# irfanfadhullah/unet_zoo

Measured on AMD Instinct MI355X. Metric: images/sec (fwd+bwd) at B=16 3x256x256, 1/2/4/8 MI355X, higher is better.
Workload: dtype bf16; 1 GPU; unet train step (zero_grad+fwd+BCE+bwd+clip+AdamW), B=16/GPU 3x256x256, random-init weights; global_batch=16, parallelism=dp1

## Files before the change

unet_zoo_amd/csrc/uz_eltwise.hip:

```cpp
#include "uz_common.h"

namespace {

template <typename T> __device__ __forceinline__ void load_f(const T* p, float* f) {
  const Vec16<T> v = ld16(p);
#pragma unroll
  for (int i = 0; i < ElemTraits<T>::VEC; ++i) f[i] = (float)v.v[i];
}
template <typename T> __device__ __forceinline__ void store_f(T* p, const float* f) {
  Vec16<T> v;
#pragma unroll
  for (int i = 0; i < ElemTraits<T>::VEC; ++i) v.v[i] = (T)f[i];
  st16(p, v);
}

template <int EW>
__global__ __launch_bounds__(1024) void bn_finalize_kernel(
    const float* __restrict__ part, int grid_m, int C, double count, const float* __restrict__ gamma,
    const float* __restrict__ beta, float eps, float momentum, float* running_mean,
    float* running_var, float* scale, float* shift, float* mean, float* invstd) {
  constexpr int NG = 1024 / EW;
  __shared__ double sh[2][NG][EW + 1];
  const int cl = threadIdx.x % EW, g = threadIdx.x / EW;
  const int c = blockIdx.x * EW + cl;
// ... 52 lines not shown
constexpr int FIN_SH_DOUBLES = 2 * 128 * 9;

template <int EW>
__device__ __forceinline__ void fin_row_sums(const float* __restrict__ part, int rows, int C, int blk, int tid, double* sh) {
  constexpr int NG = 1024 / EW, LD = EW + 1, GS = 256 / EW;
  const int cl = tid % EW, g0 = tid / EW, c = blk * EW + cl;
  double a1[4] = {0.0, 0.0, 0.0, 0.0}, a2[4] = {0.0, 0.0, 0.0, 0.0};
  if (c < C) {
    for (int r0 = g0; r0 < rows; r0 += NG) {
      float x1[4], x2[4];
#pragma unroll
      for (int k = 0; k < 4; ++k) {
        const int r = r0 + k * GS;
        const int rc = r < rows ? r : 0;
        x1[k] = part[((size_t)rc * 2 + 0) * C + c];
        x2[k] = part[((size_t)rc * 2 + 1) * C + c];
      }
#pragma unroll
      for (int k = 0; k < 4; ++k)
        if (r0 + k * GS < rows) {
          a1[k] += (double)x1[k];
          a2[k] += (double)x2[k];
        }
    }
  }
#pragma unroll
  for (int k = 0; k < 4; ++k) {
    sh[(0 * NG + g0 + k * GS) * LD + cl] = a1[k];
    sh[(1 * NG + g0 + k * GS) * LD + cl] = a2[k];
  }
  __syncthreads();
#pragma unroll
  for (int st = NG / 2; st > 0; st >>= 1) {
    for (int v = tid; v < st * EW; v += 256) {
      const int vl = v % EW, g = v / EW;
      sh[(0 * NG + g) * LD + vl] += sh[(0 * NG + g + st) * LD + vl];
      sh[(1 * NG + g) * LD + vl] += sh[(1 * NG + g + st) * LD + vl];
    }
    __syncthreads();
  }
}

struct BnFin {
  const float* part;
  int rows, ew;
  double count;
  const float *gamma, *beta;
  float eps, momentum;
  float *running_mean, *running_var;
  float* vec;
  double* sums;
  float *dgamma, *dbeta;
  int* flag;
};

#ifndef UZ_FIN_SLEEP
#define UZ_FIN_SLEEP 4
#endif
template <typename V> __device__ __forceinline__ void fin_store(V* p, V v) {
  __hip_atomic_store(p, v, __ATOMIC_RELAXED, __HIP_MEMORY_SCOPE_AGENT);
}
template <typename V> __device__ __forceinline__ V fin_load(const V* p) {
  return __hip_atomic_load(const_cast<V*>(p), __ATOMIC_RELAXED, __HIP_MEMORY_SCOPE_AGENT);
}
__device__ __forceinline__ void fin_publish(int* flag, int tid) {
  asm volatile("s_waitcnt vmcnt(0)" ::: "memory");
  __syncthreads();
  if (tid == 0) __hip_atomic_fetch_add(flag, 1, __ATOMIC_RELAXED, __HIP_MEMORY_SCOPE_AGENT);
}
__device__ __forceinline__ void fin_wait(int* flag, int nfin, int tid) {
  if (tid == 0)
    while (__hip_atomic_load(flag, __ATOMIC_RELAXED, __HIP_MEMORY_SCOPE_AGENT) < nfin) __builtin_amdgcn_s_sleep(UZ_FIN_SLEEP);
  __syncthreads();
}

template <int EW>
__device__ __forceinline__ void fin_forward(const BnFin& f, int C, int blk, int tid, double* sh) {
  constexpr int NG = 1024 / EW, LD = EW + 1;
  fin_row_sums<EW>(f.part, f.rows, C, blk, tid, sh);
  const int c = blk * EW + tid;
  if (tid < EW && c < C) {
    const double t1 = sh[(0 * NG) * LD + tid], t2 = sh[(1 * NG) * LD + tid];
    const double m = t1 / f.count;
    double var = t2 / f.count - m * m;
    if (var < 0.0) var = 0.0;
    const double istd = 1.0 / sqrt(var + (double)f.eps);
    fin_store(f.vec + c, (float)((double)f.gamma[c] * istd));
    fin_store(f.vec + C + c, (float)((double)f.beta[c] - m * (double)f.gamma[c] * istd));
    f.vec[2 * C + c] = (float)m;
    f.vec[3 * C + c] = (float)istd;
    if (f.running_mean != nullptr) {
      const double unbiased = f.count > 1.0 ? var * f.count / (f.count - 1.0) : var;
      f.running_mean[c] = (float)((1.0 - (double)f.momentum) * (double)f.running_mean[c] + (double)f.momentum * m);
      f.running_var[c] = (float)((1.0 - (double)f.momentum) * (double)f.running_var[c] + (double)f.momentum * unbiased);
    }
  }
}

template <int EW>
__device__ __forceinline__ void fin_backward(const BnFin& f, int C, int blk, int tid, double* sh) {
  constexpr int NG = 1024 / EW, LD = EW + 1;
  fin_row_sums<EW>(f.part, f.rows, C, blk, tid, sh);
  const int c = blk * EW + tid;
  if (tid < EW && c < C) {
    const double t1 = sh[(0 * NG) * LD + tid], t2 = sh[(1 * NG) * LD + tid];
    fin_store(f.sums + c, t1);
    fin_store(f.sums + C + c, t2);
    if (f.dgamma != nullptr) {
      f.dbeta[c] = (float)t1;
      f.dgamma[c] = (float)t2;
    }
  }
}

__global__ void bn_eval_scale_kernel(int C, const float* gamma, const float* beta, const float* rm,
                                     const float* rv, float eps, float* scale, float* shift) {
  const int c = blockIdx.x * blockDim.x + threadIdx.x;
  if (c < C) {
    const float istd = 1.0f / sqrtf(rv[c] + eps);
    const float sc = gamma[c] * istd;
    scale[c] = sc;
    shift[c] = beta[c] - rm[c] * sc;
  }
}

template <typename T, bool POOL, bool FIN = false>
__global__ __launch_bounds__(256) void bn_relu_apply_kernel(
    const T* __restrict__ y, int ldy, const float* scale, const float* shift,
    int N, int H, int W, int C, T* __restrict__ act, int lda, T* __restrict__ pooled, int ldp,
    const T* __restrict__ res, int ldr, int pool_ceil, const BnFin fin) {
  const float* fin_tab = nullptr;
  if constexpr (FIN) {
    __shared__ double fin_sh[FIN_SH_DOUBLES];
    const int nfin = (C + fin.ew - 1) / fin.ew;
    if ((int)blockIdx.x < nfin) {
      if (fin.ew == 8) fin_forward<8>(fin, C, blockIdx.x, threadIdx.x, fin_sh);
      else fin_forward<32>(fin, C, blockIdx.x, threadIdx.x, fin_sh);
      fin_publish(fin.flag, threadIdx.x);
    }
    fin_wait(fin.flag, nfin, threadIdx.x);
    float* tab = reinterpret_cast<float*>(fin_sh);
    for (int i = threadIdx.x; i < 2 * C; i += 256) tab[i] = fin_load(fin.vec + i);
    __syncthreads();
    fin_tab = tab;
  }
  constexpr int VEC = ElemTraits<T>::VEC;
  const int CC = C / VEC;
  const bool relu = !(pool_ceil & 2);
  const bool rev = (pool_ceil & 4) != 0;
  pool_ceil &= 1;
  const int Ho = (H + 1) >> 1, Wo = (W + 1) >> 1;
  const int Hp = pool_ceil ? Ho : H >> 1, Wp = pool_ceil ? Wo : W >> 1;
  const long long total = POOL ? (long long)N * Ho * Wo * CC : (long long)N * H * W * CC;
  for (long long idx0 = (long long)blockIdx.x * blockDim.x + threadIdx.x; idx0 < total;
       idx0 += (long long)gridDim.x * blockDim.x) {
    const long long idx = rev ? total - 1 - idx0 : idx0;
    const int cc = (int)(idx % CC);
    const long long u = idx / CC;
    const int c0 = cc * VEC;
    float sc[VEC], sh[VEC];
    if constexpr (FIN) {
#pragma unroll
      for (int i = 0; i < VEC; i += 4) {
        *reinterpret_cast<float4*>(sc + i) = *reinterpret_cast<const float4*>(fin_tab + c0 + i);
        *reinterpret_cast<float4*>(sh + i) = *reinterpret_cast<const float4*>(fin_tab + C + c0 + i);
      }
    } else {
#pragma unroll
      for (int i = 0; i < VEC; i += 4) {
        *reinterpret_cast<float4*>(sc + i) = *reinterpret_cast<const float4*>(scale + c0 + i);
        *reinterpret_cast<float4*>(sh + i) = *reinterpret_cast<const float4*>(shift + c0 + i);
      }
    }
    if constexpr (!POOL) {
      float v[VEC];
      load_f(y + (size_t)u * ldy + c0, v);
#pragma unroll
      for (int i = 0; i < VEC; ++i) {
        v[i] = fmaf(v[i], sc[i], sh[i]);
        if (relu) v[i] = fmaxf(v[i], 0.f);
      }
      if (res != nullptr) {
        float r[VEC];
        load_f(res + (size_t)u * ldr + c0, r);
#pragma unroll
        for (int i = 0; i < VEC; ++i) v[i] += r[i];
      }
      store_f(act + (size_t)u * lda + c0, v);
    } else {
      const int wo = (int)(u % Wo);
      const long long t = u / Wo;
      const int ho = (int)(t % Ho);
      const int img = (int)(t / Ho);
      const size_t p00 = ((size_t)img * H + 2 * ho) * W + 2 * wo;
      float m[VEC];
      bool ok[4];
      size_t pp[4];
      Vec16<T> vr[4], rr[4];
#pragma unroll
      for (int k = 0; k < 4; ++k) {
        ok[k] = 2 * ho + (k >> 1) < H && 2 * wo + (k & 1) < W;
        pp[k] = p00 + (k >> 1) * W + (k & 1);
        vr[k] = ld16(ok[k] ? y + pp[k] * ldy + c0 : y + c0);
        rr[k] = ld16(res != nullptr && ok[k] ? res + pp[k] * ldr + c0 : y + c0);
      }
#pragma unroll
      for (int k = 0; k < 4; ++k) {
        float v[VEC];
#pragma unroll
        for (int i = 0; i < VEC; ++i) {
          v[i] = fmaf((float)vr[k].v[i], sc[i], sh[i]);
          if (relu) v[i] = fmaxf(v[i], 0.f);
          if (res != nullptr) v[i] = (float)(T)(v[i] + (float)rr[k].v[i]);
          m[i] = (k == 0) ? v[i] : (ok[k] ? fmaxf(m[i], v[i]) : m[i]);
        }
        if (ok[k]) store_f(act + pp[k] * lda + c0, v);
      }
      if (ho < Hp && wo < Wp) store_f(pooled + (((size_t)img * Hp + ho) * Wp + wo) * ldp + c0, m);
    }
  }
}

struct BnBwdArgs {
  const void* y;
  const void* g0;
  const void* g1;
  const void* gp;
  void* dy;
  const float* scale;
  const float* shift;
  const float* mean;
  const float* invstd;
  double* sums;
  float* partials;
  float* dgamma;
  float* dbeta;
  double inv_count;
  int N, H, W, C, ldy, ldg0, ldg1, ldgp, lddy, pool_ceil;
  BnFin fin;
};

template <typename T, bool POOL, int PASS, bool FIN = false>
__global__ __launch_bounds__(256) void bn_relu_bwd_kernel(const BnBwdArgs a) {
  constexpr int VEC = ElemTraits<T>::VEC;
  const double* fin_tab = nullptr;
  if constexpr (FIN) {
    static_assert(PASS == 2, "the fused finalize belongs to the apply pass");
    __shared__ double fin_sh[FIN_SH_DOUBLES];
    const int nfin = (a.C + a.fin.ew - 1) / a.fin.ew;
    const int wg = blockIdx.y * gridDim.x + blockIdx.x, tid = threadIdx.y * blockDim.x + threadIdx.x;
    if (wg < nfin) {
      if (a.fin.ew == 8) fin_backward<8>(a.fin, a.C, wg, tid, fin_sh);
      else fin_backward<32>(a.fin, a.C, wg, tid, fin_sh);
      fin_publish(a.fin.flag, tid);
    }
    fin_wait(a.fin.flag, nfin, tid);
    const int cw = blockDim.x * VEC, cb = blockIdx.y * cw;
    for (int i = tid; i < 2 * cw; i += 256) {
      const int which = i / cw, j = i - which * cw;
      fin_sh[i] = cb + j < a.C ? fin_load(a.sums + (size_t)which * a.C + cb + j) : 0.0;
    }
    __syncthreads();
    fin_tab = fin_sh;
  }
  constexpr int NPIX = 4;
  extern __shared__ __attribute__((aligned(16))) float red[];
  const T* __restrict__ y = static_cast<const T*>(a.y);
  const T* __restrict__ g0 = static_cast<const T*>(a.g0);
  const T* __restrict__ g1 = static_cast<const T*>(a.g1);
  const T* __restrict__ gp = static_cast<const T*>(a.gp);
  T* __restrict__ dy = static_cast<T*>(a.dy);
  const int CC = a.C / VEC;
  const int cc = blockIdx.y * blockDim.x + threadIdx.x;
  const bool cok = cc < CC;
  const int c0 = (cok ? cc : 0) * VEC;
  const int Ho = (a.H + 1) >> 1, Wo = (a.W + 1) >> 1;
  const bool norelu = (a.pool_ceil & 2) != 0;
  const int Hp = (a.pool_ceil & 1) ? Ho : a.H >> 1, Wp = (a.pool_ceil & 1) ? Wo : a.W >> 1;
  const long long units = POOL ? (long long)a.N * Ho * Wo : (long long)a.N * a.H * a.W;

  float sc[VEC], sh[VEC], mu[VEC], is[VEC], k0[VEC], k1[VEC];
#pragma unroll
  for (int i = 0; i < VEC; ++i) {
    sc[i] = a.scale[c0 + i];
    sh[i] = a.shift[c0 + i];
    mu[i] = a.mean[c0 + i];
    is[i] = a.invstd[c0 + i];
    if (PASS == 2) {
      if constexpr (FIN) {
        k0[i] = (float)(fin_tab[threadIdx.x * VEC + i] * a.inv_count);
        k1[i] = (float)(fin_tab[blockDim.x * VEC + threadIdx.x * VEC + i] * a.inv_count);
      } else {
        k0[i] = (float)(a.sums[c0 + i] * a.inv_count);
        k1[i] = (float)(a.sums[a.C + c0 + i] * a.inv_count);
      }
    }
  }
  float S0[VEC], S1[VEC];
#pragma unroll
  for (int i = 0; i < VEC; ++i) S0[i] = S1[i] = 0.f;

  const long long ustride = (long long)gridDim.x * blockDim.y;
  const bool rev = (a.pool_ceil & 4) != 0;
  for (long long u0 = (long long)blockIdx.x * blockDim.y + threadIdx.y; u0 < units && cok;
       u0 += (POOL ? 1 : NPIX) * ustride) {
    size_t pix[NPIX];
    bool in[NPIX];
    size_t gpoff = 0;
    bool has_pool = false;
    if constexpr (POOL) {
      const long long u = rev ? units - 1 - u0 : u0;
      const int wo = (int)(u % Wo);
      const long long t = u / Wo;
      const int ho = (int)(t % Ho);
      const int img = (int)(t / Ho);
#pragma unroll
      for (int k = 0; k < NPIX; ++k) {
        const int hh = 2 * ho + (k >> 1), ww = 2 * wo + (k & 1);
        in[k] = hh < a.H && ww < a.W;
        pix[k] = ((size_t)img * a.H + min(hh, a.H - 1)) * a.W + min(ww, a.W - 1);
      }
      has_pool = ho < Hp && wo < Wp;
      gpoff = (((size_t)img * Hp + ho) * Wp + wo) * a.ldgp;
    } else {
#pragma unroll
      for (int k = 0; k < NPIX; ++k) {
        const long long q = u0 + k * ustride;
        in[k] = q < units;
        pix[k] = (size_t)(in[k] ? (rev ? units - 1 - q : q) : units - 1);
      }
    }
#ifndef UZ_BN_BRANCHY
    Vec16<T> yr[NPIX], g0r[NPIX], g1r[NPIX], gpr;
#pragma unroll
    for (int k = 0; k < NPIX; ++k) {
      yr[k] = ld16(y + pix[k] * a.ldy + c0);
      if constexpr (POOL) {
        g0r[k] = ld16(g0 != nullptr ? g0 + pix[k] * a.ldg0 + c0 : y + c0);
        g1r[k] = ld16(g1 != nullptr ? g1 + pix[k] * a.ldg1 + c0 : y + c0);
      } else {
        if (g0 != nullptr) g0r[k] = ld16(g0 + pix[k] * a.ldg0 + c0);
        if (g1 != nullptr) g1r[k] = ld16(g1 + pix[k] * a.ldg1 + c0);
      }
    }
    if constexpr (POOL) gpr = ld16(gp != nullptr ? gp + (has_pool ? gpoff : 0) + c0 : y + c0);
    float yv[NPIX][VEC], gv[NPIX][VEC];
#pragma unroll
    for (int k = 0; k < NPIX; ++k)
#pragma unroll
      for (int i = 0; i < VEC; ++i) {
        yv[k][i] = in[k] ? (float)yr[k].v[i] : 0.f;
        float gsum = g0 != nullptr ? (float)g0r[k].v[i] : 0.f;
        if (g1 != nullptr) gsum += (float)g1r[k].v[i];
        gv[k][i] = in[k] ? gsum : 0.f;
      }
#else
    float yv[NPIX][VEC], gv[NPIX][VEC];
#pragma unroll
    for (int k = 0; k < NPIX; ++k) {
      const size_t p = pix[k];
      if (!in[k]) {
#pragma unroll
        for (int i = 0; i < VEC; ++i) yv[k][i] = gv[k][i] = 0.f;
        continue;
      }
      load_f(y + p * a.ldy + c0, yv[k]);
      if (g0 != nullptr) {
        load_f(g0 + p * a.ldg0 + c0, gv[k]);
      } else {
#pragma unroll
        for (int i = 0; i < VEC; ++i) gv[k][i] = 0.f;
      }
      if (g1 != nullptr) {
        float t[VEC];
        load_f(g1 + p * a.ldg1 + c0, t);
#pragma unroll
        for (int i = 0; i < VEC; ++i) gv[k][i] += t[i];
      }
    }
#endif
    if constexpr (POOL) {
      if (gp != nullptr && has_pool) {
        float gpv[VEC];
#ifndef UZ_BN_BRANCHY
#pragma unroll
        for (int i = 0; i < VEC; ++i) gpv[i] = (float)gpr.v[i];
#else
        load_f(gp + gpoff + c0, gpv);
#endif
#pragma unroll
        for (int i = 0; i < VEC; ++i) {
          float best = fmaf(yv[0][i], sc[i], sh[i]);
          if (!norelu) best = fmaxf(best, 0.f);
          int bk = 0;
#pragma unroll
          for (int k = 1; k < 4; ++k) {
            float v = fmaf(yv[k][i], sc[i], sh[i]);
            if (!norelu) v = fmaxf(v, 0.f);
            if (in[k] && v > best) {
              best = v;
              bk = k;
            }
          }
#pragma unroll
          for (int k = 0; k < 4; ++k) gv[k][i] += (k == bk) ? gpv[i] : 0.f;
        }
      }
    }
#pragma unroll
    for (int k = 0; k < NPIX; ++k) {
      if (!in[k]) continue;
      float out[VEC];
#pragma unroll
      for (int i = 0; i < VEC; ++i) {
        const float pre = fmaf(yv[k][i], sc[i], sh[i]);
        const float dz = (norelu || pre > 0.f) ? gv[k][i] : 0.f;
        const float xh = (yv[k][i] - mu[i]) * is[i];
        if (PASS == 1) {
          S0[i] += dz;
          S1[i] += dz * xh;
        } else {
          out[i] = sc[i] * (dz - k0[i] - xh * k1[i]);
        }
      }
      if (PASS == 2) {
        store_f(dy + pix[k] * a.lddy + c0, out);
      }
    }
  }

  if (PASS == 1) {
    float* mine = red + ((size_t)threadIdx.y * blockDim.x + threadIdx.x) * (2 * VEC);
#pragma unroll
    for (int i = 0; i < VEC; ++i) {
      mine[i] = S0[i];
      mine[VEC + i] = S1[i];
    }
    __syncthreads();
    for (int e = threadIdx.y; e < 2 * VEC; e += blockDim.y) {
      float t = 0.f;
      for (int r = 0; r < (int)blockDim.y; ++r) t += red[((size_t)r * blockDim.x + threadIdx.x) * (2 * VEC) + e];
      if (cok) {
        const int which = e / VEC, ch = c0 + (e % VEC);
        a.partials[((size_t)blockIdx.x * 2 + which) * a.C + ch] = t;
      }
    }
  }
}

struct BnBwdHeadArgs {
  const bf16_t* y;
  bf16_t* dy;
  const float* scale;
  const float* shift;
  const float* mean;
  const float* invstd;
  const double* sums;
  const float* g;
  const float* w;
  double inv_count;
  int P, HW, C, ldy, lddy, rev;
};

template <int KOUT>
__global__ __launch_bounds__(256) void bn_relu_bwd_head_kernel(const BnBwdHeadArgs a) {
  typedef bf16_t T;
  constexpr int VEC = ElemTraits<T>::VEC, NPIX = 4;
  const T* __restrict__ y = a.y;
  const float* __restrict__ g = a.g;
  T* __restrict__ dy = a.dy;
  const int CC = a.C / VEC;
  const int cc = blockIdx.y * blockDim.x + threadIdx.x;
  const bool cok = cc < CC;
  const int c0 = (cok ? cc : 0) * VEC;
  const long long units = a.P;

  float sc[VEC], sh[VEC], mu[VEC], is[VEC], k0[VEC], k1[VEC], wr[KOUT][VEC];
#pragma unroll
  for (int i = 0; i < VEC; ++i) {
    sc[i] = a.scale[c0 + i];
    sh[i] = a.shift[c0 + i];
    mu[i] = a.mean[c0 + i];
    is[i] = a.invstd[c0 + i];
    k0[i] = (float)(a.sums[c0 + i] * a.inv_count);
    k1[i] = (float)(a.sums[a.C + c0 + i] * a.inv_count);
#pragma unroll
    for (int k = 0; k < KOUT; ++k) wr[k][i] = a.w[k * a.C + c0 + i];
  }
  const long long ustride = (long long)gridDim.x * blockDim.y;
  const bool rev = a.rev != 0;
  for (long long u0 = (long long)blockIdx.x * blockDim.y + threadIdx.y; u0 < units && cok; u0 += NPIX * ustride) {
    size_t pix[NPIX];
    bool in[NPIX];
#pragma unroll
    for (int k = 0; k < NPIX; ++k) {
      const long long q = u0 + k * ustride;
      in[k] = q < units;
      pix[k] = (size_t)(in[k] ? (rev ? units - 1 - q : q) : units - 1);
    }
    Vec16<T> yr[NPIX];
    float gq[NPIX][KOUT];
#pragma unroll
    for (int k = 0; k < NPIX; ++k) {
      yr[k] = ld16(y + pix[k] * a.ldy + c0);
      const int p = (int)pix[k];
      const int img = (KOUT == 1) ? 0 : p / a.HW;
      const int hw = p - img * a.HW;
#pragma unroll
      for (int kk = 0; kk < KOUT; ++kk) gq[k][kk] = g[((size_t)img * KOUT + kk) * a.HW + hw];
    }
#pragma unroll
    for (int k = 0; k < NPIX; ++k) {
      if (!in[k]) continue;
      float out[VEC];
#pragma unroll
      for (int i = 0; i < VEC; ++i) {
        float d = 0.f;
#pragma unroll
        for (int kk = 0; kk < KOUT; ++kk) d = fmaf(gq[k][kk], wr[kk][i], d);
        const float gv = (float)(T)d;
        const float yv = (float)yr[k].v[i];
        const float pre = fmaf(yv, sc[i], sh[i]);
        const float dz = pre > 0.f ? gv : 0.f;
        const float xh = (yv - mu[i]) * is[i];
        out[i] = sc[i] * (dz - k0[i] - xh * k1[i]);
      }
      store_f(dy + pix[k] * a.lddy + c0, out);
    }
  }
}

template <int EW>
__global__ __launch_bounds__(1024) void bn_bwd_finalize_kernel(const float* __restrict__ part, int rows,
                                                               int C, double* __restrict__ sums,
                                                               float* dgamma, float* dbeta) {
  constexpr int NG = 1024 / EW;
  __shared__ double sh[2][NG][EW + 1];
  const int cl = threadIdx.x % EW, g = threadIdx.x / EW;
  const int c = blockIdx.x * EW + cl;
  double a1 = 0.0, a2 = 0.0;
  const int cq = c < C ? c : 0;
  for (int r = g; r < rows; r += 4 * NG) {
    float p1[4], p2[4];
#pragma unroll
    for (int k = 0; k < 4; ++k) {
      const int rr = r + k * NG < rows ? r + k * NG : 0;
      p1[k] = part[((size_t)rr * 2 + 0) * C + cq];
      p2[k] = part[((size_t)rr * 2 + 1) * C + cq];
    }
#pragma unroll
    for (int k = 0; k < 4; ++k) asm volatile("" : "+v"(p1[k]), "+v"(p2[k]));
#pragma unroll
    for (int k = 0; k < 4; ++k)
      if (r + k * NG < rows && c < C) {
        a1 += (double)p1[k];
        a2 += (double)p2[k];
      }
  }
  sh[0][g][cl] = a1;
  sh[1][g][cl] = a2;
  __syncthreads();
#pragma unroll
  for (int st = NG / 2; st > 0; st >>= 1) {
    if (g < st) {
      sh[0][g][cl] += sh[0][g + st][cl];
      sh[1][g][cl] += sh[1][g + st][cl];
    }
    __syncthreads();
  }
  if (g == 0 && c < C) {
    const double t1 = sh[0][0][cl], t2 = sh[1][0][cl];
    sums[c] = t1;
    sums[C + c] = t2;
    if (dgamma != nullptr) {
      dbeta[c] = (float)t1;
      dgamma[c] = (float)t2;
    }
  }
}

constexpr int OUTCONV_MAXK = 8;
__host__ __device__ inline int lanes_per_pixel(int chunks) {
  int l = 1;
  while (l < chunks) l <<= 1;
  return l;
}

template <typename T, int KOUT, bool XF = false>
__global__ __launch_bounds__(256) void outconv_fwd_kernel(const T* __restrict__ x, int ldx, int N,
                                                          int HW, int C, const float* __restrict__ w,
                                                          const float* __restrict__ b,
                                                          float* __restrict__ out,
                                                          const float* __restrict__ xf_scale = nullptr,
                                                          const float* __restrict__ xf_shift = nullptr) {
  constexpr int VEC = ElemTraits<T>::VEC;
  const int LPP = lanes_per_pixel(C / VEC);
  const int ppb = blockDim.x / LPP;
  const int sub = threadIdx.x % LPP, pl = threadIdx.x / LPP;
  const bool live = sub < C / VEC;
  const int P = N * HW;
  float wr[KOUT][VEC];
#pragma unroll
  for (int k = 0; k < KOUT; ++k)
#pragma unroll
    for (int i = 0; i < VEC; ++i) wr[k][i] = live ? w[k * C + sub * VEC + i] : 0.f;
  float xsc[VEC], xsh[VEC];
  if constexpr (XF) {
#pragma unroll
    for (int i = 0; i < VEC; ++i) {
      xsc[i] = live ? xf_scale[sub * VEC + i] : 0.f;
      xsh[i] = live ? xf_shift[sub * VEC + i] : 0.f;
    }
  }
  for (int p0 = blockIdx.x * ppb; p0 < P; p0 += gridDim.x * ppb) {
    const int p = p0 + pl;
    float v[VEC];
    if (p < P && live) {
      load_f(x + (size_t)p * ldx + sub * VEC, v);
      if constexpr (XF) {
#pragma unroll
        for (int i = 0; i < VEC; ++i) v[i] = (float)(T)fmaxf(fmaf(v[i], xsc[i], xsh[i]), 0.f);
      }
    } else {
#pragma unroll
      for (int i = 0; i < VEC; ++i) v[i] = 0.f;
    }
    const int img = (KOUT == 1) ? 0 : p / HW;
    const int hw = p - img * HW;
#pragma unroll
    for (int k = 0; k < KOUT; ++k) {
      float s = 0.f;
#pragma unroll
      for (int i = 0; i < VEC; ++i) s = fmaf(v[i], wr[k][i], s);
      for (int o = LPP >> 1; o > 0; o >>= 1) s += __shfl_xor(s, o);
      if (sub == 0 && p < P) out[((size_t)img * KOUT + k) * HW + hw] = s + b[k];
    }
  }
}

template <typename T, int KOUT, bool BNRED = false, bool XNULL = false>
__global__ __launch_bounds__(256) void outconv_bwd_kernel(const T* __restrict__ x, int ldx, int N,
                                                          int HW, int C, const float* __restrict__ w,
                                                          const float* __restrict__ g,
                                                          T* __restrict__ dx, int lddx,
                                                          float* __restrict__ partial, const T* __restrict__ bn_y = nullptr, int ld_bny = 0,
                                                          const float* __restrict__ bn_scale = nullptr, const float* __restrict__ bn_shift = nullptr,
                                                          const float* __restrict__ bn_mean = nullptr, const float* __restrict__ bn_invstd = nullptr,
                                                          float* __restrict__ bnpart = nullptr) {
  constexpr int VEC = ElemTraits<T>::VEC;
// ... 373 lines not shown
      {
        float tv[16];
#pragma unroll
        for (int k = 0; k < 16; ++k) {
          const int r = ty + 4 * k;
          tv[k] = src[(r0 + r < R && c0 + tx < Cc) ? (size_t)(r0 + r) * Cc + c0 + tx : 0];
        }
#pragma unroll
        for (int k = 0; k < 16; ++k) asm volatile("" : "+v"(tv[k]));
#pragma unroll
        for (int k = 0; k < 16; ++k) {
          const int r = ty + 4 * k;
          tile[r][tx] = (r0 + r < R && c0 + tx < Cc) ? tv[k] : 0.f;
        }
      }
      __syncthreads();
      for (int c = ty; c < 64; c += 4)
        if (c0 + c < Cc && r0 + tx < R) dst[(size_t)(c0 + c) * R + r0 + tx] = (T)tile[tx][c];
    }
    return;
  }
  if (it.T == 4 && it.mode == UZ_PACK_CONVT_DGRAD && count == 4LL * it.Co * it.Ci) {
    const int rowlen = 4 * it.Co;
    for (int ci = blockIdx.x; ci < it.Ci; ci += gridDim.x) {
      const float* __restrict__ srow = src + (size_t)ci * rowlen;
      T* __restrict__ drow = dst + (size_t)ci * rowlen;
      for (int k = threadIdx.x; k < rowlen; k += 256) {
        const int t = k / it.Co, co = k - t * it.Co;
        drow[k] = (T)srow[4 * co + t];
      }
    }
    return;
  }
  if (it.T == 4 && it.mode == UZ_PACK_CONVT_FWD && count == 4LL * it.Co * it.Ci) {
    const int R = it.Ci, Cc = 4 * it.Co;
    __shared__ float tile4[64][65];
    const int tr = (R + 63) / 64, tc = (Cc + 63) / 64;
    const int tx = threadIdx.x & 63, ty = threadIdx.x >> 6;
    for (int t = blockIdx.x; t < tr * tc; t += gridDim.x) {
      const int r0 = (t / tc) * 64, c0 = (t % tc) * 64;
      __syncthreads();
      {
        float tv[16];
#pragma unroll
        for (int k = 0; k < 16; ++k) {
          const int r = ty + 4 * k;
          tv[k] = src[(r0 + r < R && c0 + tx < Cc) ? (size_t)(r0 + r) * Cc + c0 + tx : 0];
        }
#pragma unroll
        for (int k = 0; k < 16; ++k) asm volatile("" : "+v"(tv[k]));
#pragma unroll
        for (int k = 0; k < 16; ++k) {
          const int r = ty + 4 * k;
          tile4[r][tx] = (r0 + r < R && c0 + tx < Cc) ? tv[k] : 0.f;
        }
      }
      __syncthreads();
      for (int c = ty; c < 64; c += 4) {
        const int j = c0 + c;
        if (j < Cc && r0 + tx < R) dst[(size_t)((j & 3) * it.Co + (j >> 2)) * R + r0 + tx] = (T)tile4[tx][c];
      }
    }
    return;
  }
  for (long long idx = (long long)blockIdx.x * blockDim.x + threadIdx.x; idx < count;
       idx += (long long)gridDim.x * blockDim.x)
    dst[idx] = (T)pack_element(it.mode, it.src, it.Co, it.Ci, it.T, it.Kpad, idx);
}

template <typename T>
__global__ void im2col3x3_kernel(const float* __restrict__ x, int N, int C, int H, int W, int Kpad,
                                 T* __restrict__ dst, long long total) {
  constexpr int VEC = ElemTraits<T>::VEC;
  const int cpr = Kpad / VEC;
  for (long long idx = (long long)blockIdx.x * blockDim.x + threadIdx.x; idx < total;
       idx += (long long)gridDim.x * blockDim.x) {
    const int ch = (int)(idx % cpr);
    const long long p = idx / cpr;
    const int w0 = (int)(p % W);
    const long long q = p / W;
    const int h0 = (int)(q % H);
    const int img = (int)(q / H);
    Vec16<T> v;
#pragma unroll
    for (int e = 0; e < VEC; ++e) {
      const int k = ch * VEC + e;
      float f = 0.f;
      if (k < 9 * C) {
        const int t = k / C, c = k - t * C;
        const int hh = h0 + t / 3 - 1, ww = w0 + t % 3 - 1;
        if ((unsigned)hh < (unsigned)H && (unsigned)ww < (unsigned)W)
          f = x[(((size_t)img * C + c) * H + hh) * W + ww];
      }
      v.v[e] = (T)f;
    }
    st16(dst + (size_t)p * Kpad + ch * VEC, v);
  }
}

template <typename T, int C>
__global__ __launch_bounds__(256) void im2col3x3_smallc_kernel(const float* __restrict__ x, int N, int H,
                                                               int W, int Kpad, T* __restrict__ dst,
                                                               long long npix) {
  constexpr int VEC = ElemTraits<T>::VEC;
  constexpr int K = 9 * C;
  constexpr int MAXCH = 64 / VEC;
  constexpr int ROWB = MAXCH * 16 + 16;
  __shared__ __attribute__((aligned(16))) char strip[4][64 * ROWB];
  const int nch = Kpad / VEC;
  const int lane = threadIdx.x & 63, wv = threadIdx.x >> 6;
  char* mine = strip[wv];
  for (long long p0 = ((long long)blockIdx.x * blockDim.x + (threadIdx.x & ~63)); p0 < npix;
       p0 += (long long)gridDim.x * blockDim.x) {
    const long long p = p0 + lane;
    float row[K];
    if (p < npix) {
      const int w0 = (int)(p % W);
      const long long q = p / W;
      const int h0 = (int)(q % H);
      const int img = (int)(q / H);
#pragma unroll
      for (int t = 0; t < 9; ++t) {
        const int hh = h0 + t / 3 - 1, ww = w0 + t % 3 - 1;
        const bool ok = (unsigned)hh < (unsigned)H && (unsigned)ww < (unsigned)W;
#pragma unroll
        for (int c = 0; c < C; ++c) row[t * C + c] = ok ? x[(((size_t)img * C + c) * H + hh) * W + ww] : 0.f;
      }
    } else {
#pragma unroll
      for (int k = 0; k < K; ++k) row[k] = 0.f;
    }
#pragma unroll
    for (int ch = 0; ch < MAXCH; ++ch) {
      if (ch < nch) {
        Vec16<T> v;
#pragma unroll
        for (int e = 0; e < VEC; ++e) v.v[e] = (ch * VEC + e < K) ? (T)row[(ch * VEC + e < K) ? ch * VEC + e : 0] : (T)0.f;
        *reinterpret_cast<Vec16<T>*>(mine + lane * ROWB + ch * 16) = v;
      }
    }
    asm volatile("s_waitcnt lgkmcnt(0)" ::: "memory");
    const int total = 64 * nch;
    for (int j = lane; j < total; j += 64) {
      const int px = j / nch, ch = j - px * nch;
      if (p0 + px < npix) {
        const Vec16<T> v = *reinterpret_cast<const Vec16<T>*>(mine + px * ROWB + ch * 16);
        st16(dst + (size_t)(p0 + px) * Kpad + ch * VEC, v);
      }
    }
    asm volatile("s_waitcnt lgkmcnt(0)" ::: "memory");
  }
}

int grid_for(long long total, int block) {
  long long g = (total + block - 1) / block;
  const long long cap = (long long)UZ_NUM_CU * 8;
  if (g > cap) g = cap;
  if (g < 1) g = 1;
  return (int)g;
}


void reduce_shape(int CC, long long units, dim3* grid, dim3* block, int wg_per_cu = 2) {
  int bx = 1;
  while (bx < CC && bx < 64) bx <<= 1;
  const int by = 256 / bx;
  const int gy = (CC + bx - 1) / bx;
  long long gx = (units + by - 1) / by;
  long long cap = (long long)UZ_NUM_CU * wg_per_cu / gy;
  if (cap < 1) cap = 1;
  if (gx > cap) gx = cap;
  if (gx < 1) gx = 1;
  *grid = dim3((unsigned)gx, (unsigned)gy);
  *block = dim3(bx, by);
}

}

extern "C" int uz_bn_finalize(const float* stats_partial, int grid_m, int C, double count,
                              const float* gamma, const float* beta, float eps, float momentum,
                              float* running_mean, float* running_var, float* scale, float* shift,
                              float* mean, float* invstd, void* stream) {
  UZ_REQUIRE(stats_partial && gamma && beta && scale && shift && mean && invstd, "uz_bn_finalize: null");
  UZ_REQUIRE(grid_m > 0 && C > 0 && count > 0, "uz_bn_finalize: bad shape");
  UZ_REQUIRE((running_mean == nullptr) == (running_var == nullptr), "uz_bn_finalize: running stats");
  if (grid_m >= 128 && C <= 512)
    hipLaunchKernelGGL(bn_finalize_kernel<8>, dim3(uz_cdiv(C, 8)), dim3(1024), 0, (hipStream_t)stream,
                       stats_partial, grid_m, C, count, gamma, beta, eps, momentum, running_mean,
                       running_var, scale, shift, mean, invstd);
  else
    hipLaunchKernelGGL(bn_finalize_kernel<32>, dim3(uz_cdiv(C, 32)), dim3(1024), 0, (hipStream_t)stream,
                       stats_partial, grid_m, C, count, gamma, beta, eps, momentum, running_mean,
                       running_var, scale, shift, mean, invstd);
  UZ_LAUNCH_CHECK("uz_bn_finalize");
  return UZ_OK;
}

extern "C" int uz_bn_eval_scale(int C, const float* gamma, const float* beta, const float* running_mean,
                                const float* running_var, float eps, float* scale, float* shift,
                                void* stream) {
  UZ_REQUIRE(C > 0 && gamma && beta && running_mean && running_var && scale && shift, "uz_bn_eval_scale: null");
  hipLaunchKernelGGL(bn_eval_scale_kernel, dim3(uz_cdiv(C, 256)), dim3(256), 0, (hipStream_t)stream, C,
                     gamma, beta, running_mean, running_var, eps, scale, shift);
  UZ_LAUNCH_CHECK("uz_bn_eval_scale");
  return UZ_OK;
}

template <typename T>
static int bn_relu_apply_t(const void* y, int ldy, const float* scale, const float* shift, int N, int H,
                           int W, int C, void* act, int lda, void* pooled, int ldp, const void* res, int ldr,
                           int pool_ceil, hipStream_t s) {
  constexpr int VEC = ElemTraits<T>::VEC;
  if (pooled != nullptr) {
    const long long total = (long long)N * ((H + 1) / 2) * ((W + 1) / 2) * (C / VEC);
    hipLaunchKernelGGL((bn_relu_apply_kernel<T, true>), dim3(grid_for(total, 256)), dim3(256), 0, s,
                       (const T*)y, ldy, scale, shift, N, H, W, C, (T*)act, lda, (T*)pooled, ldp, (const T*)res, ldr, pool_ceil, BnFin{});
  } else {
    const long long total = (long long)N * H * W * (C / VEC);
    hipLaunchKernelGGL((bn_relu_apply_kernel<T, false>), dim3(grid_for(total, 256)), dim3(256), 0, s,
                       (const T*)y, ldy, scale, shift, N, H, W, C, (T*)act, lda, (T*)nullptr, 0, (const T*)res, ldr, pool_ceil & 6, BnFin{});
  }
  UZ_LAUNCH_CHECK("uz_bn_relu_apply");
  return UZ_OK;
}

extern "C" int uz_bn_relu_add_apply(int dtype, const void* y, int ldy, const float* scale, const float* shift,
                                    int N, int H, int W, int C, const void* res, int ldr, void* act, int lda,
                                    void* pooled, int ldp, int pool_ceil, void* stream);

extern "C" int uz_bn_relu_apply(int dtype, const void* y, int ldy, const float* scale, const float* shift,
                                int N, int H, int W, int C, void* act, int lda, void* pooled, int ldp,
                                void* stream) {
  return uz_bn_relu_add_apply(dtype, y, ldy, scale, shift, N, H, W, C, nullptr, 0, act, lda, pooled, ldp, 0, stream);
}

extern "C" int uz_bn_relu_add_apply(int dtype, const void* y, int ldy, const float* scale, const float* shift,
                                    int N, int H, int W, int C, const void* res, int ldr, void* act, int lda,
                                    void* pooled, int ldp, int pool_ceil, void* stream) {
  UZ_REQUIRE(dtype == UZ_F32 || dtype == UZ_BF16, "uz_bn_relu_apply: bad dtype");
  const int vec = dtype == UZ_BF16 ? 8 : 4;
  UZ_REQUIRE(y && scale && shift && act, "uz_bn_relu_apply: null pointer");
  UZ_REQUIRE(N > 0 && H > 0 && W > 0 && C > 0 && C % vec == 0, "uz_bn_relu_apply: C=%d must be a multiple of %d", C, vec);
  UZ_REQUIRE(ldy % vec == 0 && lda % vec == 0 && ldy >= C && lda >= C, "uz_bn_relu_apply: bad ld");
  if (res != nullptr) UZ_REQUIRE(ldr % vec == 0 && ldr >= C, "uz_bn_relu_apply: bad ldr");
  if (pooled != nullptr) {
    UZ_REQUIRE((pool_ceil & 1) || (H >= 2 && W >= 2), "uz_bn_relu_apply: floor-mode pool of a %dx%d map is empty", H, W);
    UZ_REQUIRE(ldp % vec == 0 && ldp >= C, "uz_bn_relu_apply: bad ldp");
  }
  hipStream_t s = (hipStream_t)stream;
  return dtype == UZ_BF16 ? bn_relu_apply_t<bf16_t>(y, ldy, scale, shift, N, H, W, C, act, lda, pooled, ldp, res, ldr, pool_ceil, s)
                          : bn_relu_apply_t<float>(y, ldy, scale, shift, N, H, W, C, act, lda, pooled, ldp, res, ldr, pool_ceil, s);
}

static inline int fin_ew(int rows, int C) { return (rows >= 128 && C <= 512) ? 8 : 32; }

template <typename T>
static int bn_relu_apply_fin_t(const void* y, int ldy, const BnFin& fin, int N, int H, int W, int C, void* act, int lda,
                               void* pooled, int ldp, const void* res, int ldr, int pool_ceil, hipStream_t s, bool* done) {
  constexpr int VEC = ElemTraits<T>::VEC;
  const bool pool = pooled != nullptr;
  const long long total = (pool ? (long long)N * ((H + 1) / 2) * ((W + 1) / 2) : (long long)N * H * W) * (C / VEC);
  const int grid = grid_for(total, 256);
  *done = grid >= (C + fin.ew - 1) / fin.ew && 2 * C <= 2 * FIN_SH_DOUBLES;
  if (!*done) return UZ_OK;
  if (pool)
    hipLaunchKernelGGL((bn_relu_apply_kernel<T, true, true>), dim3(grid), dim3(256), 0, s, (const T*)y, ldy, fin.vec, fin.vec + C, N,
                       H, W, C, (T*)act, lda, (T*)pooled, ldp, (const T*)res, ldr, pool_ceil, fin);
  else
    hipLaunchKernelGGL((bn_relu_apply_kernel<T, false, true>), dim3(grid), dim3(256), 0, s, (const T*)y, ldy, fin.vec, fin.vec + C,
                       N, H, W, C, (T*)act, lda, (T*)nullptr, 0, (const T*)res, ldr, pool_ceil & 6, fin);
  UZ_LAUNCH_CHECK("uz_bn_relu_add_apply_fin");
  return UZ_OK;
}

extern "C" int uz_bn_relu_add_apply_fin(int dtype, const void* y, int ldy, const float* stats_partial, int rows, double count,
                                        const float* gamma, const float* beta, float eps, float momentum, float* running_mean,
                                        float* running_var, float* vec, int* flag, int N, int H, int W, int C, const void* res,
                                        int ldr, void* act, int lda, void* pooled, int ldp, int pool_ceil, void* stream) {
  UZ_REQUIRE(dtype == UZ_F32 || dtype == UZ_BF16, "uz_bn_relu_add_apply_fin: bad dtype");
  const int vecw = dtype == UZ_BF16 ? 8 : 4;
  UZ_REQUIRE(y && act && stats_partial && gamma && beta && vec && flag, "uz_bn_relu_add_apply_fin: null pointer");
  UZ_REQUIRE(rows > 0 && count > 0, "uz_bn_relu_add_apply_fin: bad statistics shape");
  UZ_REQUIRE((running_mean == nullptr) == (running_var == nullptr), "uz_bn_relu_add_apply_fin: running stats");
  UZ_REQUIRE(N > 0 && H > 0 && W > 0 && C > 0 && C % vecw == 0, "uz_bn_relu_add_apply_fin: C=%d must be a multiple of %d", C, vecw);
  UZ_REQUIRE(ldy % vecw == 0 && lda % vecw == 0 && ldy >= C && lda >= C, "uz_bn_relu_add_apply_fin: bad ld");
  if (res != nullptr) UZ_REQUIRE(ldr % vecw == 0 && ldr >= C, "uz_bn_relu_add_apply_fin: bad ldr");
  if (pooled != nullptr) {
    UZ_REQUIRE((pool_ceil & 1) || (H >= 2 && W >= 2), "uz_bn_relu_add_apply_fin: floor-mode pool of a %dx%d map is empty", H, W);
    UZ_REQUIRE(ldp % vecw == 0 && ldp >= C, "uz_bn_relu_add_apply_fin: bad ldp");
  }
  BnFin fin{};
  fin.part = stats_partial; fin.rows = rows; fin.ew = fin_ew(rows, C); fin.count = count;
  fin.gamma = gamma; fin.beta = beta; fin.eps = eps; fin.momentum = momentum;
  fin.running_mean = running_mean; fin.running_var = running_var; fin.vec = vec; fin.flag = flag;
  hipStream_t s = (hipStream_t)stream;
  bool done = false;
  const int rc = dtype == UZ_BF16
      ? bn_relu_apply_fin_t<bf16_t>(y, ldy, fin, N, H, W, C, act, lda, pooled, ldp, res, ldr, pool_ceil, s, &done)
      : bn_relu_apply_fin_t<float>(y, ldy, fin, N, H, W, C, act, lda, pooled, ldp, res, ldr, pool_ceil, s, &done);
  if (rc != UZ_OK || done) return rc;
  const int rc2 = uz_bn_finalize(stats_partial, rows, C, count, gamma, beta, eps, momentum, running_mean, running_var, vec,
                                 vec + C, vec + 2 * C, vec + 3 * C, stream);
  if (rc2 != UZ_OK) return rc2;
  return uz_bn_relu_add_apply(dtype, y, ldy, vec, vec + C, N, H, W, C, res, ldr, act, lda, pooled, ldp, pool_ceil, stream);
}

static int bnbwd_check(const uz_bnbwd_desc* d, const void* g0, const void* g1, const void* gp) {
  UZ_REQUIRE(d != nullptr, "uz_bn_relu_bwd: null descriptor");
  UZ_REQUIRE(d->dtype == UZ_F32 || d->dtype == UZ_BF16, "uz_bn_relu_bwd: bad dtype");
  const int vec = d->dtype == UZ_BF16 ? 8 : 4;
  UZ_REQUIRE(d->N > 0 && d->H > 0 && d->W > 0 && d->C > 0 && d->C % vec == 0, "uz_bn_relu_bwd: bad shape");
  UZ_REQUIRE(d->ldy % vec == 0 && d->ldy >= d->C, "uz_bn_relu_bwd: bad ldy");
  if (g0) UZ_REQUIRE(d->ldg0 % vec == 0 && d->ldg0 >= d->C, "uz_bn_relu_bwd: bad ldg0");
  if (g1) UZ_REQUIRE(d->ldg1 % vec == 0 && d->ldg1 >= d->C, "uz_bn_relu_bwd: bad ldg1");
  if (gp) {
    UZ_REQUIRE(d->ldgp % vec == 0 && d->ldgp >= d->C, "uz_bn_relu_bwd: bad ldgp");
  }
  UZ_REQUIRE(g0 || g1 || gp, "uz_bn_relu_bwd: no incoming gradient");
  return UZ_OK;
}

static void bnbwd_shape(const uz_bnbwd_desc* d, bool pool, dim3* grid, dim3* block, int pass = 1) {
  const int vec = d->dtype == UZ_BF16 ? 8 : 4;
  const long long units = pool ? (long long)d->N * ((d->H + 1) / 2) * ((d->W + 1) / 2) : (long long)d->N * d->H * d->W;
  const int f = uz_tune_flags() & 6;
  reduce_shape(d->C / vec, units, grid, block, pass == 2 ? 8 : (f == 2 ? 8 : f == 4 ? 6 : 4));
}

template <typename T, int PASS, bool FIN = false>
static int bnbwd_launch(const uz_bnbwd_desc* d, const BnBwdArgs& a, bool pool, hipStream_t s) {
  constexpr int VEC = ElemTraits<T>::VEC;
  dim3 grid, block;
  bnbwd_shape(d, pool, &grid, &block, PASS);
  const size_t shm = PASS == 1 ? (size_t)256 * 2 * VEC * sizeof(float) : 0;
  if constexpr (FIN) {
    UZ_REQUIRE((long long)grid.x * grid.y >= (a.C + a.fin.ew - 1) / a.fin.ew && block.x * block.y == 256,
               "uz_bn_relu_bwd_apply_fin: the grid is smaller than the finalize (ask uz_bn_relu_bwd_apply_fin_supported)");
  }
  if (pool) {
    hipLaunchKernelGGL((bn_relu_bwd_kernel<T, true, PASS, FIN>), grid, block, shm, s, a);
  } else {
    hipLaunchKernelGGL((bn_relu_bwd_kernel<T, false, PASS, FIN>), grid, block, shm, s, a);
  }
  UZ_LAUNCH_CHECK("uz_bn_relu_bwd");
  return UZ_OK;
}

static BnBwdArgs bnbwd_args(const uz_bnbwd_desc* d, const void* y, const float* scale, const float* shift,
                            const float* mean, const float* invstd, const void* g0, const void* g1,
                            const void* gp) {
  BnBwdArgs a;
  a.y = y;
  a.g0 = g0;
  a.g1 = g1;
  a.gp = gp;
  a.dy = nullptr;
  a.scale = scale;
  a.shift = shift;
  a.mean = mean;
  a.invstd = invstd;
  a.sums = nullptr;
  a.partials = nullptr;
  a.dgamma = nullptr;
  a.dbeta = nullptr;
  a.inv_count = 0.0;
  a.N = d->N;
  a.H = d->H;
  a.W = d->W;
  a.C = d->C;
  a.ldy = d->ldy;
  a.ldg0 = d->ldg0;
  a.ldg1 = d->ldg1;
  a.ldgp = d->ldgp;
  a.pool_ceil = d->pool_ceil;
  a.lddy = d->lddy;
  a.fin = BnFin{};
  return a;
}

static void bnbwd_finalize(const float* partial, int rows, int C, double* sums, float* dgamma, float* dbeta,
                           hipStream_t s) {
  if (rows >= 128 && C <= 512)
    hipLaunchKernelGGL(bn_bwd_finalize_kernel<8>, dim3(uz_cdiv(C, 8)), dim3(1024), 0, s, partial, rows, C, sums, dgamma, dbeta);
  else
    hipLaunchKernelGGL(bn_bwd_finalize_kernel<32>, dim3(uz_cdiv(C, 32)), dim3(1024), 0, s, partial, rows, C, sums, dgamma, dbeta);
}

extern "C" long long uz_bn_relu_bwd_workspace_bytes(const uz_bnbwd_desc* d, int has_pool_grad) {
  UZ_REQUIRE(d != nullptr && d->C > 0 && d->N > 0 && d->H > 0 && d->W > 0, "uz_bn_relu_bwd_workspace_bytes: bad descriptor");
  UZ_REQUIRE(d->dtype == UZ_F32 || d->dtype == UZ_BF16, "uz_bn_relu_bwd_workspace_bytes: bad dtype");
  dim3 grid, block;
  bnbwd_shape(d, has_pool_grad != 0, &grid, &block);
  return (long long)grid.x * 2 * d->C * (long long)sizeof(float);
}

extern "C" int uz_bn_relu_bwd_reduce(const uz_bnbwd_desc* d, const void* y, const float* scale,
                                     const float* shift, const float* mean, const float* invstd,
                                     const void* g0, const void* g1, const void* gpool, void* workspace,
                                     double* sums, float* dgamma, float* dbeta, void* stream) {
  const int rc = bnbwd_check(d, g0, g1, gpool);
  if (rc != UZ_OK) return rc;
  UZ_REQUIRE(y && scale && shift && mean && invstd && sums && workspace, "uz_bn_relu_bwd_reduce: null pointer");
  UZ_REQUIRE((dgamma == nullptr) == (dbeta == nullptr), "uz_bn_relu_bwd_reduce: dgamma/dbeta");
  BnBwdArgs a = bnbwd_args(d, y, scale, shift, mean, invstd, g0, g1, gpool);
  a.partials = static_cast<float*>(workspace);
  hipStream_t s = (hipStream_t)stream;
  const int rc2 = d->dtype == UZ_BF16 ? bnbwd_launch<bf16_t, 1>(d, a, gpool != nullptr, s)
                                      : bnbwd_launch<float, 1>(d, a, gpool != nullptr, s);
  if (rc2 != UZ_OK) return rc2;
  dim3 grid, block;
  bnbwd_shape(d, gpool != nullptr, &grid, &block);
  bnbwd_finalize(static_cast<const float*>(workspace), (int)grid.x, d->C, sums, dgamma, dbeta, s);
  UZ_LAUNCH_CHECK("uz_bn_relu_bwd_reduce(finalize)");
  return UZ_OK;
}

extern "C" int uz_bn_bwd_finalize(const float* partial, int rows, int C, double* sums, float* dgamma, float* dbeta,
                                  void* stream) {
  UZ_REQUIRE(partial && sums && rows > 0 && C > 0, "uz_bn_bwd_finalize: bad arguments");
  UZ_REQUIRE((dgamma == nullptr) == (dbeta == nullptr), "uz_bn_bwd_finalize: dgamma/dbeta");
  bnbwd_finalize(partial, rows, C, sums, dgamma, dbeta, (hipStream_t)stream);
  UZ_LAUNCH_CHECK("uz_bn_bwd_finalize");
  return UZ_OK;
}

extern "C" int uz_bn_relu_bwd_apply(const uz_bnbwd_desc* d, const void* y, const float* scale,
                                    const float* shift, const float* mean, const float* invstd,
                                    const void* g0, const void* g1, const void* gpool, const double* sums,
                                    double count, void* dy, void* stream) {
  const int rc = bnbwd_check(d, g0, g1, gpool);
  if (rc != UZ_OK) return rc;
  UZ_REQUIRE(y && scale && shift && mean && invstd && sums && dy, "uz_bn_relu_bwd_apply: null pointer");
  UZ_REQUIRE(count > 0, "uz_bn_relu_bwd_apply: count");
  const int vec = d->dtype == UZ_BF16 ? 8 : 4;
  UZ_REQUIRE(d->lddy % vec == 0 && d->lddy >= d->C, "uz_bn_relu_bwd_apply: bad lddy");
  BnBwdArgs a = bnbwd_args(d, y, scale, shift, mean, invstd, g0, g1, gpool);
  a.sums = const_cast<double*>(sums);
  a.dy = dy;
  a.inv_count = 1.0 / count;
  hipStream_t s = (hipStream_t)stream;
  return d->dtype == UZ_BF16 ? bnbwd_launch<bf16_t, 2>(d, a, gpool != nullptr, s)
                             : bnbwd_launch<float, 2>(d, a, gpool != nullptr, s);
}

extern "C" int uz_bn_relu_bwd_reduce_rows(const uz_bnbwd_desc* d, const void* y, const float* scale, const float* shift,
                                          const float* mean, const float* invstd, const void* g0, const void* g1,
                                          const void* gpool, void* workspace, void* stream) {
  const int rc = bnbwd_check(d, g0, g1, gpool);
  if (rc != UZ_OK) return rc;
  UZ_REQUIRE(y && scale && shift && mean && invstd && workspace, "uz_bn_relu_bwd_reduce_rows: null pointer");
  BnBwdArgs a = bnbwd_args(d, y, scale, shift, mean, invstd, g0, g1, gpool);
  a.partials = static_cast<float*>(workspace);
  hipStream_t s = (hipStream_t)stream;
  return d->dtype == UZ_BF16 ? bnbwd_launch<bf16_t, 1>(d, a, gpool != nullptr, s) : bnbwd_launch<float, 1>(d, a, gpool != nullptr, s);
}

extern "C" int uz_bn_relu_bwd_apply_fin(const uz_bnbwd_desc* d, const void* y, const float* scale, const float* shift,
                                        const float* mean, const float* invstd, const void* g0, const void* g1,
                                        const void* gpool, const float* partial, int rows, double* sums, float* dgamma,
                                        float* dbeta, int* flag, double count, void* dy, void* stream) {
  const int rc = bnbwd_check(d, g0, g1, gpool);
  if (rc != UZ_OK) return rc;
  UZ_REQUIRE(y && scale && shift && mean && invstd && sums && dy && partial && flag, "uz_bn_relu_bwd_apply_fin: null pointer");
  UZ_REQUIRE(count > 0 && rows > 0, "uz_bn_relu_bwd_apply_fin: count / rows");
  UZ_REQUIRE((dgamma == nullptr) == (dbeta == nullptr), "uz_bn_relu_bwd_apply_fin: dgamma/dbeta");
  const int vec = d->dtype == UZ_BF16 ? 8 : 4;
  UZ_REQUIRE(d->lddy % vec == 0 && d->lddy >= d->C, "uz_bn_relu_bwd_apply_fin: bad lddy");
  BnBwdArgs a = bnbwd_args(d, y, scale, shift, mean, invstd, g0, g1, gpool);
  a.sums = sums;
  a.dy = dy;
  a.inv_count = 1.0 / count;
  a.fin.part = partial; a.fin.rows = rows; a.fin.ew = fin_ew(rows, d->C);
  a.fin.sums = sums; a.fin.dgamma = dgamma; a.fin.dbeta = dbeta; a.fin.flag = flag;
  hipStream_t s = (hipStream_t)stream;
  dim3 grid, block;
  bnbwd_shape(d, gpool != nullptr, &grid, &block, 2);
  if ((long long)grid.x * grid.y < (d->C + a.fin.ew - 1) / a.fin.ew) {
    bnbwd_finalize(partial, rows, d->C, sums, dgamma, dbeta, s);
    UZ_LAUNCH_CHECK("uz_bn_relu_bwd_apply_fin(finalize)");
// ... 527 lines not shown
```

Before: 2503 images/sec.

## Specialize BN-ReLU apply fast path and make bwd pixel batches adjacent

Adds a non-pool, non-finalize fast path to the BN+ReLU apply kernel. When the block size is a multiple of the channel-vector count, each thread loads its scale/shift once, and the per-element division becomes a shift. The pass-2 and fused-conv backward kernels now place their NPIX pixels adjacent within a block rather than a grid-stride apart, and the pass-2 grid is sized for a quarter of the units. The pooled apply launch also allows more workgroups per CU. These changes aim to cut index arithmetic and redundant table loads and to improve memory locality, at the cost of more code paths and a shift that assumes CC is a power of two.

```diff
diff --git a/unet_zoo_amd/csrc/uz_eltwise.hip b/unet_zoo_amd/csrc/uz_eltwise.hip
--- a/unet_zoo_amd/csrc/uz_eltwise.hip
+++ b/unet_zoo_amd/csrc/uz_eltwise.hip
@@ -228,6 +228,46 @@
   const int Ho = (H + 1) >> 1, Wo = (W + 1) >> 1;
   const int Hp = pool_ceil ? Ho : H >> 1, Wp = pool_ceil ? Wo : W >> 1;
   const long long total = POOL ? (long long)N * Ho * Wo * CC : (long long)N * H * W * CC;
+  if constexpr (!POOL && !FIN) {
+    const bool fixed_cc = (int)blockDim.x % CC == 0;
+    const int cc_shift = __ffs(CC) - 1;
+    float sc[VEC], sh[VEC];
+    auto table = [&](int c0) {
+#pragma unroll
+      for (int i = 0; i < VEC; i += 4) {
+        *reinterpret_cast<float4*>(sc + i) = *reinterpret_cast<const float4*>(scale + c0 + i);
+        *reinterpret_cast<float4*>(sh + i) = *reinterpret_cast<const float4*>(shift + c0 + i);
+      }
+    };
+    int my_c0 = 0;
+    if (fixed_cc) {
+      const int t = (int)threadIdx.x % CC;
+      my_c0 = (rev ? CC - 1 - t : t) * VEC;
+      table(my_c0);
+    }
+    for (long long idx0 = (long long)blockIdx.x * blockDim.x + threadIdx.x; idx0 < total;
+         idx0 += (long long)gridDim.x * blockDim.x) {
+      const long long idx = rev ? total - 1 - idx0 : idx0;
+      const int c0 = fixed_cc ? my_c0 : (int)(idx % CC) * VEC;
+      const long long u = fixed_cc ? idx >> cc_shift : idx / CC;
+      const Vec16<T> vr = ld16(y + (size_t)u * ldy + c0);
+      Vec16<T> rr;
+      if (res != nullptr) rr = ld16(res + (size_t)u * ldr + c0);
+      if (!fixed_cc) table(c0);
+      float v[VEC];
+#pragma unroll
+      for (int i = 0; i < VEC; ++i) {
+        v[i] = fmaf((float)vr.v[i], sc[i], sh[i]);
+        if (relu) v[i] = fmaxf(v[i], 0.f);
+      }
+      if (res != nullptr) {
+#pragma unroll
+        for (int i = 0; i < VEC; ++i) v[i] += (float)rr.v[i];
+      }
+      store_f(act + (size_t)u * lda + c0, v);
+    }
+    return;
+  }
   for (long long idx0 = (long long)blockIdx.x * blockDim.x + threadIdx.x; idx0 < total;
        idx0 += (long long)gridDim.x * blockDim.x) {
     const long long idx = rev ? total - 1 - idx0 : idx0;
@@ -378,7 +418,9 @@
 
   const long long ustride = (long long)gridDim.x * blockDim.y;
   const bool rev = (a.pool_ceil & 4) != 0;
-  for (long long u0 = (long long)blockIdx.x * blockDim.y + threadIdx.y; u0 < units && cok;
+  constexpr bool ADJ = !POOL && PASS == 2;
+  const long long kstep = ADJ ? (long long)blockDim.y : ustride;
+  for (long long u0 = (long long)blockIdx.x * blockDim.y * (ADJ ? NPIX : 1) + threadIdx.y; u0 < units && cok;
        u0 += (POOL ? 1 : NPIX) * ustride) {
     size_t pix[NPIX];
     bool in[NPIX];
@@ -401,7 +443,7 @@
     } else {
 #pragma unroll
       for (int k = 0; k < NPIX; ++k) {
-        const long long q = u0 + k * ustride;
+        const long long q = u0 + k * kstep;
         in[k] = q < units;
         pix[k] = (size_t)(in[k] ? (rev ? units - 1 - q : q) : units - 1);
       }
@@ -565,12 +607,13 @@
   }
   const long long ustride = (long long)gridDim.x * blockDim.y;
   const bool rev = a.rev != 0;
-  for (long long u0 = (long long)blockIdx.x * blockDim.y + threadIdx.y; u0 < units && cok; u0 += NPIX * ustride) {
+  const long long kstep = blockDim.y;
+  for (long long u0 = (long long)blockIdx.x * blockDim.y * NPIX + threadIdx.y; u0 < units && cok; u0 += NPIX * ustride) {
     size_t pix[NPIX];
     bool in[NPIX];
 #pragma unroll
     for (int k = 0; k < NPIX; ++k) {
-      const long long q = u0 + k * ustride;
+      const long long q = u0 + k * kstep;
       in[k] = q < units;
       pix[k] = (size_t)(in[k] ? (rev ? units - 1 - q : q) : units - 1);
     }
@@ -1250,9 +1293,9 @@
   }
 }
 
-int grid_for(long long total, int block) {
+int grid_for(long long total, int block, int wg_per_cu = 8) {
   long long g = (total + block - 1) / block;
-  const long long cap = (long long)UZ_NUM_CU * 8;
+  const long long cap = (long long)UZ_NUM_CU * wg_per_cu;
   if (g > cap) g = cap;
   if (g < 1) g = 1;
   return (int)g;
@@ -1311,7 +1354,7 @@
   constexpr int VEC = ElemTraits<T>::VEC;
   if (pooled != nullptr) {
     const long long total = (long long)N * ((H + 1) / 2) * ((W + 1) / 2) * (C / VEC);
-    hipLaunchKernelGGL((bn_relu_apply_kernel<T, true>), dim3(grid_for(total, 256)), dim3(256), 0, s,
+    hipLaunchKernelGGL((bn_relu_apply_kernel<T, true>), dim3(grid_for(total, 256, 32)), dim3(256), 0, s,
                        (const T*)y, ldy, scale, shift, N, H, W, C, (T*)act, lda, (T*)pooled, ldp, (const T*)res, ldr, pool_ceil, BnFin{});
   } else {
     const long long total = (long long)N * H * W * (C / VEC);
@@ -1422,7 +1465,8 @@
   const int vec = d->dtype == UZ_BF16 ? 8 : 4;
   const long long units = pool ? (long long)d->N * ((d->H + 1) / 2) * ((d->W + 1) / 2) : (long long)d->N * d->H * d->W;
   const int f = uz_tune_flags() & 6;
-  reduce_shape(d->C / vec, units, grid, block, pass == 2 ? 8 : (f == 2 ? 8 : f == 4 ? 6 : 4));
+  if (pass == 2 && !pool) reduce_shape(d->C / vec, (units + 3) / 4, grid, block, 8);
+  else reduce_shape(d->C / vec, units, grid, block, pass == 2 ? 8 : (f == 2 ? 8 : f == 4 ? 6 : 4));
 }
 
 template <typename T, int PASS, bool FIN = false>
```

Result: no change. 2523 images/sec (median of 6 runs) (+0.8%).
